# DeepGraphLearning/ULTRA

Measured on AMD Instinct MI355X. Metric: triples scored/sec (all-tail ranking) on FB15k237, higher is better.
Workload: dtype f32

## Files before the change

ultra_amd/build.py:

```python
import concurrent.futures as cf
import glob
import os
import subprocess
import sys

HERE = os.path.dirname(os.path.abspath(__file__))
CSRC = os.path.join(HERE, "csrc")
LIB_DIR = os.path.join(HERE, "lib")
OBJ_DIR = os.path.join(LIB_DIR, "obj")
LIB = os.path.join(LIB_DIR, "libultra_amd.so")
INCLUDE = os.path.join(os.path.dirname(HERE), "include")

HIPCC = os.environ.get("HIPCC", "/opt/rocm/bin/hipcc")
ARCH = "gfx950"
CFLAGS = ["--offload-arch=" + ARCH, "-O3", "-std=c++17", "-fPIC", "-ffp-contract=off",
          "-munsafe-fp-atomics", "-Wall", "-Wno-unused-function", "-I" + INCLUDE]


def _sources():
    return sorted(glob.glob(os.path.join(CSRC, "*.hip")) + glob.glob(os.path.join(CSRC, "*.cpp")))


def _headers_mtime():
    hs = glob.glob(os.path.join(CSRC, "*.hpp")) + glob.glob(os.path.join(INCLUDE, "*.h"))
    return max(os.path.getmtime(h) for h in hs)


def _compile(src, obj):
    cmd = [HIPCC] + CFLAGS + ["-c", src, "-o", obj]
    if src.endswith(".cpp"):
        cmd = [HIPCC] + CFLAGS + ["-x", "hip", "-c", src, "-o", obj]
    r = subprocess.run(cmd, capture_output=True, text=True)
    if r.returncode != 0:
        raise RuntimeError("hipcc failed for %s:\n%s\n%s" % (src, r.stdout, r.stderr))
    return r.stderr


def build(force=False, verbose=False):
    os.makedirs(OBJ_DIR, exist_ok=True)
    hm = _headers_mtime()
    jobs = []
    objs = []
    for src in _sources():
        obj = os.path.join(OBJ_DIR, os.path.basename(src) + ".o")
        objs.append(obj)
        stale = force or not os.path.exists(obj) or os.path.getmtime(obj) < max(os.path.getmtime(src), hm)
        if stale:
            jobs.append((src, obj))
    if jobs:
        with cf.ThreadPoolExecutor(max_workers=min(8, os.cpu_count() or 1)) as ex:
            futs = {ex.submit(_compile, s, o): s for s, o in jobs}
            for f in cf.as_completed(futs):
                warn = f.result()
                if verbose and warn.strip():
# ... 52 lines not shown
```

ultra_amd/csrc/plan.cpp:

```cpp
#include "plan.hpp"

#include <algorithm>
#include <cstdio>
#include <cstdlib>
#include <cstring>
#include <numeric>
#include <queue>

namespace ultra {

static thread_local std::string g_last_error;

void set_error(const std::string &msg) { g_last_error = msg; }

static int bits_for(int64_t n) {
    int b = 0;
    while ((int64_t(1) << b) < n) ++b;
    return b;
}

static void counting_pass(std::vector<int32_t> &order, const int32_t *key, int64_t nkey) {
    const int64_t n = (int64_t)order.size();
    std::vector<int64_t> start((size_t)nkey + 1, 0);
    for (int64_t i = 0; i < n; ++i) start[(size_t)key[order[i]] + 1]++;
// ... 102 lines not shown
            const int32_t t = p->type[(size_t)k], r = p->erow[(size_t)k];
            if (last_row[(size_t)t] != r) {
                last_row[(size_t)t] = r;
                ++runs;
            }
        }
        p->n_type_run = runs;
    }

    if (exact) {
        p->rec.resize((size_t)E * 2);
        for (int64_t k = 0; k < E; ++k) {
            p->rec[(size_t)2 * k] = p->col[(size_t)k];
            p->rec[(size_t)2 * k + 1] = p->type[(size_t)k];
        }
    }

    std::vector<Item> witems, gitems, chain;
    int32_t next_slot = 0;
    p->split_ptr.push_back(0);
    for (int64_t r = 0; r < num_out; ++r) {
        const int32_t b = p->row_ptr[(size_t)r], e = p->row_ptr[(size_t)r + 1];
        const int32_t deg = e - b;
        if (type_runs) {
            std::vector<Item> mine;
            int32_t pos = b;
            while (pos < e) {
                int32_t end = pos + 1;
                while (end < e && p->type[(size_t)end] == p->type[(size_t)pos]) ++end;
                const int32_t len_run = end - pos;
// ... 207 lines not shown
            sload[(size_t)stream] += p->items[(size_t)g].len + 1;
            scost[(size_t)stream] += p->items[(size_t)g].len + 1 + (walkers == 12 ? ROW_COST_12[(stream % ORDER_GROUPS) / 16] : 0.0);
        };
        {
        for (int64_t g = 0; g < nstream; ++g)
            if (weight[(size_t)g] > 0.0) sheap.push(Slot(1.0 / weight[(size_t)g], g));
        for (int64_t g = 0; g < n_item; ++g) {
            if (g < n_chain && !to_stream[(size_t)g]) continue;
            const Slot sl = sheap.top();
            sheap.pop();
            deal_into(sl.second, g);
            sheap.push(Slot((scost[(size_t)sl.second] + 1.0) / weight[(size_t)sl.second], sl.second));
        }
        }
        s->sdesc.assign((size_t)nstream * 2, 0);
        s->srec.reserve((size_t)(2 * (int64_t)steps) + 2 * ORDER_PAD);
        for (int64_t g = 0; g < nstream; ++g) {
            s->sdesc[(size_t)2 * g] = (int32_t)(s->srec.size() / 2);
            s->sdesc[(size_t)2 * g + 1] = (int32_t)sload[(size_t)g];
            s->max_stream_steps = std::max<int32_t>(s->max_stream_steps, (int32_t)sload[(size_t)g]);
            static const int row_order_env = std::getenv("ULTRA_STREAM_ROW_ORDER") ? std::atoi(std::getenv("ULTRA_STREAM_ROW_ORDER")) : -1;
            const int row_order = row_order_env >= 0 ? row_order_env : (walkers == 12 ? 2 : 0);
            std::sort(srows[(size_t)g].begin(), srows[(size_t)g].end(), [&](int32_t a, int32_t b) {
                const Item &ia = p->items[(size_t)a], &ib = p->items[(size_t)b];
                if (row_order == 1 && ia.len != ib.len) return ia.len > ib.len;
                if (row_order == 2 && ia.len != ib.len) return ia.len < ib.len;
                return ia.row < ib.row;
            });
            const int shift = (walkers == 12 && ULTRA_STREAM_PRESHIFT) ? 8 : 0;
            s->rec_shift = shift;
            for (int32_t it : srows[(size_t)g]) {
                const Item &row = p->items[(size_t)it];
                for (int32_t e = row.begin; e < row.begin + row.len; ++e) {
                    s->srec.push_back((int32_t)((uint32_t)p->col[(size_t)e] << shift));
                    s->srec.push_back((int32_t)((uint32_t)p->type[(size_t)e] << shift));
                }
                s->srec.push_back((int32_t)((uint32_t)row.row << shift));
                s->srec.push_back((int32_t)((uint32_t)p->num_rel << shift));
            }
        }
        s->srec_pad = 2 * ((int64_t)ORDER_PAD + (int64_t)s->max_stream_steps);
        s->srec.resize(s->srec.size() + (size_t)s->srec_pad, 0);
        s->prow_ptr.assign((size_t)nparts + 1, 0);
        for (int32_t q = 0; q < nparts; ++q) {
            std::vector<int32_t> mine;
            for (int32_t c : part_chain[(size_t)q]) mine.push_back(p->items[(size_t)c].row);
            for (int g = 0; g < ORDER_GROUPS; ++g)
                for (int32_t it : srows[(size_t)q * ORDER_GROUPS + g]) mine.push_back(p->items[(size_t)it].row);
            std::sort(mine.begin(), mine.end());
            s->prow.insert(s->prow.end(), mine.begin(), mine.end());
            while (s->prow.size() % 32) s->prow.push_back(-1);
            s->prow_ptr[(size_t)q + 1] = (int32_t)s->prow.size();
            s->max_rows = std::max<int32_t>(s->max_rows, (int32_t)mine.size());
            s->max_chain_rows = std::max<int32_t>(s->max_chain_rows, (int32_t)part_chain[(size_t)q].size());
        }
    }
// ... 62 lines not shown
        set_error("ultra_plan_get_info: NULL argument");
        return ULTRA_ERR_INVALID;
    }
    info->num_edge = p->num_edge;
    info->num_node = p->num_out;
    info->num_relation = p->num_rel;
    info->n_item = (int64_t)p->items.size();
    info->n_wave_item = p->n_w;
    info->n_group_item = p->n_g;
    info->n_unit = p->n_unit;
    info->n_split_row = (int64_t)p->split_row.size();
    info->n_partial_slot = p->n_slot;
    info->seg_len = p->seg_len;
    info->g_max = p->g_max;
    info->flags = p->flags;
    info->packed = p->packed_ok ? 1 : 0;
    info->on_device = p->on_device ? 1 : 0;
    info->has_transpose = (p->tplan && p->rplan) ? 1 : 0;
    info->n_type_run = p->n_type_run;
    info->dense_bytes = (int64_t)p->a_frag.size();
    info->n_chain_row = p->n_chain;
    info->dense_order_bytes = (int64_t)p->a_ex.size();
    return ULTRA_OK;
}

int32_t ultra_plan_export(const ultra_plan *p, int32_t which, void *dst, int64_t capacity, int64_t *count) {
    if (!p || !count) {
        set_error("ultra_plan_export: NULL argument");
        return ULTRA_ERR_INVALID;
    }
    const void *src = nullptr;
// ... 26 lines not shown
```

ultra_amd/csrc/plan.hpp:

```cpp
#pragma once

#include <cstdint>
#include <map>
#include <mutex>
#include <string>
#include <vector>

#include "../../include/ultra_rspmm.h"

namespace ultra {

struct Item {
    int32_t row, begin, len, slot;
};

struct Chunk {
    int32_t row, begin, count, flags;
};
enum { CHUNK_FIRST = 1, CHUNK_LAST = 2, CHUNK_LEN_SHIFT = 2 };
#ifndef ULTRA_ORDER_WAVES
#define ULTRA_ORDER_WAVES 16
#endif
constexpr int ORDER_WAVES = ULTRA_ORDER_WAVES;
constexpr int CHAIN_SLOTS = 4 * (ORDER_WAVES - 1);
constexpr int ORDER_GROUPS = 4 * ORDER_WAVES;
constexpr int CHUNK_PAD = 32;
#ifndef ULTRA_STREAM_PRESHIFT
#define ULTRA_STREAM_PRESHIFT 1
#endif
constexpr int ORDER_PAD = 128;

struct Schedule {
    int32_t nparts = 0;
    std::vector<int32_t> chunk_ptr, unit_ptr, units;
    std::vector<Chunk> chunks;
    std::vector<int32_t> srec, sdesc;
    std::vector<int32_t> prow, prow_ptr;
    int32_t *d_chunk_ptr = nullptr, *d_unit_ptr = nullptr, *d_units = nullptr, *d_srec = nullptr, *d_sdesc = nullptr;
    int32_t *d_prow = nullptr, *d_prow_ptr = nullptr;
    Chunk *d_chunks = nullptr;
    double max_cost = 0.0, mean_cost = 0.0;
    int32_t max_rows = 0;
    int32_t max_chain_rows = 0;
    int32_t max_stream_steps = 0;
    int32_t rec_shift = 0;
    int64_t srec_pad = 2 * ORDER_PAD;
};

struct WeightCopy {
    void *buf = nullptr;
    size_t bytes = 0;
    int64_t epoch = 0;
    const void *src = nullptr;
    int32_t dtype = -1;
    void *stream = nullptr;
    unsigned long long cap_id = 0;
};

struct DevicePlan {
    int32_t *row_ptr = nullptr, *col = nullptr, *type = nullptr, *perm = nullptr, *erow = nullptr;
    int32_t *rec = nullptr;
    uint32_t *packed = nullptr;
    Item *items = nullptr;
    int32_t *split_row = nullptr, *split_ptr = nullptr;
    uint8_t *a_frag = nullptr;
    uint8_t *a16 = nullptr;
    uint8_t *a_ex = nullptr;
    uint8_t *self_loop = nullptr;
    WeightCopy w_copy[2];
    void *partial = nullptr;
    size_t partial_bytes = 0;
    void *rb_rec_c = nullptr, *rb_seg_c = nullptr, *rb_multi_c = nullptr;
    void *rb_rec_t = nullptr, *rb_seg_t = nullptr, *rb_multi_t = nullptr;
    void *rb_work = nullptr;
    size_t rb_work_bytes = 0;
    int device = -1;
// ... 9 lines not shown
    int64_t num_edge = 0, num_out = 0, num_in = 0, num_rel = 0;
    int32_t seg_len = 256, g_max = 64, flags = 0;
    int32_t type_bits = 0;
    bool packed_ok = false;
    int32_t max_row_len = -1;
    bool rb_built = false;
    int64_t rb_n_seg_c = 0, rb_n_multi_c = 0, rb_n_part_c = 0, rb_n_seg_t = 0, rb_n_multi_t = 0, rb_n_part_t = 0;

    std::vector<int32_t> row_ptr, col, type, perm, erow;
    std::vector<uint32_t> packed;
    std::vector<ultra::Item> items;
    int64_t n_w = 0, n_g = 0, n_unit = 0;
    int64_t n_chain = 0;
    int32_t chain_min = 256;
    std::vector<int32_t> rec;
    std::map<int32_t, ultra::Schedule *> schedules;
    std::mutex sched_mu;
    std::vector<int32_t> split_row, split_ptr;
    int64_t n_slot = 0;
    int64_t n_type_run = 0;

    std::vector<uint8_t> a_frag;
    int32_t dense_rt = 0, dense_kg = 0, dense_tc = 0, dense_ntc = 0;
    bool dense_overflow = false;
    std::vector<uint8_t> a16;
    int32_t a16_chunks = 0;
    std::vector<uint8_t> a_ex;

    std::vector<uint8_t> self_loop;

// ... 20 lines not shown
```

ultra_amd/csrc/rspmm_api.hip:

```cpp
#include <hip/hip_runtime.h>

#include <cstdio>
#include <cstring>
#include <functional>
#include <string>
#include <vector>

#include "device_scope.hpp"
#include "layer0_kernels.hpp"
#include "rspmm_bwd_kernels.hpp"
#include "rspmm_kernels.hpp"
#include "rspmm_order_kernels.hpp"
#include "rspmm_rows_kernels.hpp"
#include "rows_bwd_kernels.hpp"

namespace ultra {

#define ULTRA_EXTERN_VARIANT(T_, VEC_, MODE_) \
    template <>                               \
    hipError_t launch_fwd_variant<T_, VEC_, MODE_>(int, int, const FwdParams &, int, int, size_t, hipStream_t);
ULTRA_EXTERN_VARIANT(float, 4, 0)
ULTRA_EXTERN_VARIANT(float, 1, 0)
ULTRA_EXTERN_VARIANT(float, 4, 1)
ULTRA_EXTERN_VARIANT(float, 4, 2)
// ... 114 lines not shown
    if (p->flags & ULTRA_PLAN_DENSE) {
        if ((rc = upload_array(&p->d.a_frag, p->a_frag))) return rc;
        if (!p->a16.empty() && (rc = upload_array(&p->d.a16, p->a16))) return rc;
        if (!p->a_ex.empty() && (rc = upload_array(&p->d.a_ex, p->a_ex))) return rc;
        p->d.device = dev;
        p->on_device = true;
        return ULTRA_OK;
    }
    if ((rc = upload_array(&p->d.row_ptr, p->row_ptr))) return rc;
    if ((rc = upload_array(&p->d.col, p->col))) return rc;
    if ((rc = upload_array(&p->d.type, p->type))) return rc;
    if (p->flags & ULTRA_PLAN_EXACT_ORDER) {
        int64_t longest = 0;
        for (size_t i = (size_t)p->n_chain; i < p->items.size(); ++i) longest = std::max<int64_t>(longest, p->items[i].len);
        const size_t pad = (size_t)ORDER_PAD + (size_t)std::min<int64_t>(longest, 1 << 20);
        std::vector<int32_t> perm_pad(p->perm), rec_pad(p->rec);
        perm_pad.resize(p->perm.size() + pad, 0);
        rec_pad.resize(p->rec.size() + 2 * pad, 0);
        if ((rc = upload_array(&p->d.perm, perm_pad))) return rc;
        if ((rc = upload_array(&p->d.rec, rec_pad))) return rc;
    } else if ((rc = upload_array(&p->d.perm, p->perm))) {
        return rc;
    }
    if ((rc = upload_array(&p->d.erow, p->erow))) return rc;
    if ((rc = upload_array(&p->d.packed, p->packed))) return rc;
    if ((rc = upload_array(&p->d.items, p->items))) return rc;
    if ((rc = upload_array(&p->d.split_row, p->split_row))) return rc;
    if ((rc = upload_array(&p->d.split_ptr, p->split_ptr))) return rc;
    if (!p->self_loop.empty() && (rc = upload_array(&p->d.self_loop, p->self_loop))) return rc;
    p->d.device = dev;
    p->on_device = true;
    return ULTRA_OK;
}

static void free_schedules(ultra_plan *p) {
    std::lock_guard<std::mutex> lock(p->sched_mu);
    for (auto &kv : p->schedules) {
        Schedule *s = kv.second;
        if (s->d_chunk_ptr) (void)hipFree(s->d_chunk_ptr);
        if (s->d_unit_ptr) (void)hipFree(s->d_unit_ptr);
        if (s->d_units) (void)hipFree(s->d_units);
        if (s->d_chunks) (void)hipFree(s->d_chunks);
        if (s->d_srec) (void)hipFree(s->d_srec);
        if (s->d_sdesc) (void)hipFree(s->d_sdesc);
        if (s->d_prow) (void)hipFree(s->d_prow);
        if (s->d_prow_ptr) (void)hipFree(s->d_prow_ptr);
        delete s;
// ... 22 lines not shown
    *out = s;
    return ULTRA_OK;
}

static void free_device(ultra_plan *p) {
    free_schedules(p);
    if (!p->on_device) return;
    (void)hipFree(p->d.row_ptr);
    (void)hipFree(p->d.col);
    (void)hipFree(p->d.type);
    (void)hipFree(p->d.perm);
    (void)hipFree(p->d.erow);
    (void)hipFree(p->d.packed);
    (void)hipFree(p->d.items);
    if (p->d.rec) (void)hipFree(p->d.rec);
    (void)hipFree(p->d.split_row);
    (void)hipFree(p->d.split_ptr);
    if (p->d.a_frag) (void)hipFree(p->d.a_frag);
    if (p->d.a16) (void)hipFree(p->d.a16);
    if (p->d.a_ex) (void)hipFree(p->d.a_ex);
    if (p->d.self_loop) (void)hipFree(p->d.self_loop);
    for (WeightCopy &c : p->d.w_copy)
        if (c.buf) (void)hipFree(c.buf);
    if (p->d.partial) (void)hipFree(p->d.partial);
    for (void *q : {p->d.rb_rec_c, p->d.rb_seg_c, p->d.rb_multi_c, p->d.rb_rec_t, p->d.rb_seg_t, p->d.rb_multi_t, p->d.rb_work})
        if (q) (void)hipFree(q);
    p->rb_built = false;
    p->d = DevicePlan();
    p->on_device = false;
}
// ... 153 lines not shown
    op->upd.mode = 1;
    *lds = std::max(*lds, (size_t)UPDATE_LDS_FLOATS * sizeof(float));
    Schedule *sched12 = nullptr;
    const bool pitch_ok = !ULTRA_STREAM_PRESHIFT || op->x_row_bytes == 256u;
    const bool walk_heavy = (double)(p->num_edge + p->num_out) >= 10.0 * (double)p->num_out;
    const bool want3 = update_form() == 3 || (update_form() == 0 && walk_heavy);
    if (want3 && pitch_ok && ORDER_WAVES == 16 && upd->out_stride_row * (int64_t)sizeof(float) == (int64_t)op->x_row_bytes) {
        if ((rc = get_schedule(p, op->nparts, &sched12, ORDER_WALKERS))) return rc;
        const size_t overlay = std::max(ring_bytes, (size_t)UPD2_OVERLAY_BYTES);
        const size_t need = rel_bytes + overlay + UPD2_CTL_BYTES;
        if (need <= di.lds_optin && sched12->max_chain_rows <= UPD2_MAX_CHAIN_ROWS) {
            op->upd.mode = 3;
            op->max_stream_steps = sched12->max_stream_steps;
            op->upd.ctl_off = (uint32_t)(rel_bytes + overlay);
            op->srec = sched12->d_srec;
            op->sdesc = reinterpret_cast<const int2 *>(sched12->d_sdesc);
            op->chunk_ptr = sched12->d_chunk_ptr;
            op->chunks = reinterpret_cast<const int4 *>(sched12->d_chunks);
            *lds = need;
        }
    }
    if (update_form() == 2) {
        set_error("ultra_rspmm_forward_update: update form 2 (rows by reference) was removed in ABI 6; ask for 0 (the library's "
                  "choice), 1 (tail) or 3 (beside the walk, rows through LDS)");
        return ULTRA_ERR_UNSUPPORTED;
    }
    if (update_form() >= 2 && op->upd.mode != update_form()) {
        set_error("ultra_rspmm_forward_update: the update beside the walk does not fit this call (LDS / rows per workgroup)");
        return ULTRA_ERR_UNSUPPORTED;
    }
// ... 40 lines not shown
                         const ultra_mat *out, hipStream_t stream, const FwdCall &call, const FwdParams &fp, const DevInfo &di,
                         size_t ring_bytes, bool point_fill) {
    const size_t esz = dtype == ULTRA_F32 ? 4 : 8;
    const int64_t row_len = out->row_len;
    const int64_t *bnd_rows = call.bnd_rows;
    int rc;
    const size_t rel_bytes = (mul != BIN_RHS) ? (size_t)(p->num_rel + 1) * 64 * esz : 0;
    const bool rel_lds = g_tuning.rel_lds != 0 && rel_bytes > 0 && rel_bytes + ring_bytes <= di.lds_optin;
    const int grid = launch_grid(di);
    OrderParams op;
    std::memset(&op, 0, sizeof(op));
    op.smod = std::min<int32_t>(fp.n_span, grid);
    op.nparts = grid / op.smod;
    Schedule *sched = nullptr;
    if ((rc = get_schedule(p, op.nparts, &sched))) return rc;
    op.rec = p->d.rec;
    op.perm = p->d.perm;
    op.w = w;
    op.items = reinterpret_cast<const int4 *>(p->d.items);
    op.unit_ptr = sched->d_unit_ptr;
    op.units = sched->d_units;
    op.chunk_ptr = sched->d_chunk_ptr;
    op.chunks = reinterpret_cast<const int4 *>(sched->d_chunks);
    op.n_chain = (int32_t)p->n_chain;
    op.n_item = (int32_t)p->items.size();
    op.rel = fp.rel, op.x = fp.x, op.bnd = fp.bnd;
    op.bnd_rows = fp.bnd_rows;
    op.bnd_fill_on = point_fill ? 1 : 0;
    op.bnd_fill = 0.f;
    op.out = fp.out;
    op.out_stride_outer = fp.out_stride_outer, op.out_stride_row = fp.out_stride_row;
    op.n_outer = fp.n_outer, op.row_len = fp.row_len, op.spans_per_outer = fp.spans_per_outer, op.n_span = fp.n_span;
    op.num_rel = fp.num_rel;
    op.has_bnd = fp.has_bnd;
    op.has_chain = p->n_chain > 0 ? 1 : 0;
    op.keep_mode = fp.keep_mode;
    op.w_stride_outer = (w && call.w_samples) ? (int32_t)call.w_stride_outer : 0;
    op.x_row_bytes = fp.x_row_bytes, op.rel_row_bytes = fp.rel_row_bytes;
    op.trace = g_order_trace;
    op.err = device_error_word();
    op.srec = sched->d_srec;
    op.sdesc = reinterpret_cast<const int2 *>(sched->d_sdesc);
    op.use_streams = (unit_walk() == 0 && dtype == ULTRA_F32 && rel_lds && !w && (mul == BIN_MUL || mul == BIN_ADD) &&
                      row_len % 64 == 0 && (!bnd || bnd_rows) && out->stride_row == x->stride_row &&
                      p->num_out <= p->num_in && (uint64_t)p->num_out * (uint64_t)out->stride_row * esz < (1ull << 32))
                         ? 1
                         : 0;
    size_t lds = (rel_lds ? rel_bytes : 0) + ring_bytes;
    if (call.upd && (rc = choose_update_form(p, call.upd, sched, di, rel_bytes, ring_bytes, &op, &lds))) return rc;
    if (call.ev_before) HIP_TRY(hipEventRecord(call.ev_before, stream));
#define ULTRA_ORDER_LAUNCH(T_)                                                                          \
    (rel_lds ? (w ? launch_order_variant<T_, true, true>(sum, mul, op, grid, lds, stream)                \
                  : launch_order_variant<T_, true, false>(sum, mul, op, grid, lds, stream))              \
             : (w ? launch_order_variant<T_, false, true>(sum, mul, op, grid, lds, stream)               \
                  : launch_order_variant<T_, false, false>(sum, mul, op, grid, lds, stream)))
    const hipError_t e = dtype == ULTRA_F32 ? ULTRA_ORDER_LAUNCH(float) : ULTRA_ORDER_LAUNCH(double);
#undef ULTRA_ORDER_LAUNCH
    if (e != hipSuccess) return hip_fail(e, "rspmm_order_kernel launch");
    if (call.ev_after) HIP_TRY(hipEventRecord(call.ev_after, stream));
    return ULTRA_OK;
}

static int forward_walk(ultra_plan *p, int sum, int mul, int dtype, const void *w, const ultra_mat *bnd, const ultra_mat *out,
                        hipStream_t stream, const FwdCall &call, FwdParams &fp, const DevInfo &di, int VEC, bool rot_far) {
// ... 1034 lines not shown

int32_t ultra_plan_schedule_export(ultra_plan *plan, int32_t nparts, int32_t which, int32_t *dst, int64_t capacity, int64_t *count) {
    const int32_t walkers = (nparts & ULTRA_SCHEDULE_12_WALKERS) ? 12 : 16;
    nparts &= ~ULTRA_SCHEDULE_12_WALKERS;
    if (!plan || !count || nparts <= 0) return invalid("ultra_plan_schedule_export: bad argument");
    if (!(plan->flags & ULTRA_PLAN_EXACT_ORDER)) return invalid("schedules belong to ULTRA_PLAN_EXACT_ORDER plans");
    Schedule *s = build_schedule(plan, nparts, walkers);
    const int32_t *src = nullptr;
    int64_t n = 0;
    switch (which) {
        case 0: src = s->chunk_ptr.data(), n = (int64_t)s->chunk_ptr.size(); break;
        case 1: src = s->unit_ptr.data(), n = (int64_t)s->unit_ptr.size(); break;
        case 2: src = s->units.data(), n = (int64_t)s->units.size(); break;
        case 3: src = reinterpret_cast<const int32_t *>(s->chunks.data()), n = (int64_t)s->chunk_ptr.back() * 4; break;
        case 4: src = s->sdesc.data(), n = (int64_t)s->sdesc.size(); break;
        case 5: src = s->srec.data(), n = (int64_t)s->srec.size() - s->srec_pad; break;
        case 6: src = s->prow.data(), n = (int64_t)s->prow.size(); break;
        case 7: src = s->prow_ptr.data(), n = (int64_t)s->prow_ptr.size(); break;
        default: delete s; return invalid("ultra_plan_schedule_export: unknown array id");
    }
    *count = n;
    int rc = ULTRA_OK;
    if (dst) {
        if (capacity < n) rc = invalid("ultra_plan_schedule_export: destination too small");
        else if (n) std::memcpy(dst, src, (size_t)n * sizeof(int32_t));
        if (rc == ULTRA_OK && which == 5 && s->rec_shift)
            for (int64_t i = 0; i < n; ++i) dst[i] = (int32_t)((uint32_t)dst[i] >> s->rec_shift);
    }
    delete s;
    return rc;
}

int32_t ultra_device_error(void) { return take_device_error(); }

int32_t ultra_set_tuning(const ultra_tuning *t) {
    if (!t) {
        g_tuning = ultra_tuning{0, 0, -1, -1, 0, {0, 0, 0}};
        return ULTRA_OK;
    }
// ... 57 lines not shown
```

ultra_amd/csrc/rspmm_order_kernels.hpp:

```cpp
#pragma once

#include "rspmm_kernels.hpp"
#ifdef ULTRA_ORDER_ASM_HEADER
#include ULTRA_ORDER_ASM_HEADER
#else
#include "rspmm_order_asm.hpp"
#endif
#include "update_tile.hpp"

static_assert(ULTRA_STREAM_PRESHIFT_GEN == ULTRA_STREAM_PRESHIFT,
              "the generated walk and plan.cpp must agree on the record format of the twelve-walker schedules (plan.hpp)");

#pragma clang fp contract(off)

namespace ultra {

constexpr int ORDER_THREADS = 64 * ORDER_WAVES;
constexpr uint32_t SPIN_CAP = 1u << 20;
enum { ORDER_SPIN_LOOK = 1,
       ORDER_SPIN_MEET = 2,
       ORDER_SPIN_CHAIN_WALKER = 3,
       ORDER_SPIN_CHAIN_UPDATER = 4,
       ORDER_SPIN_PARK = 5 };
constexpr int ORDER_UPDATERS = 4, ORDER_WALKERS = ORDER_THREADS / 64 - ORDER_UPDATERS;
#ifndef ULTRA_CHAIN_PRIO
#define ULTRA_CHAIN_PRIO 1
#endif
static_assert(CHAIN_SLOTS == 4 * (ORDER_THREADS / 64 - 1), "one ring slot per producer group");

struct OrderParams {
    const int32_t *rec;
    const int32_t *perm;
    const void *w;
    const int4 *items;
    const int32_t *unit_ptr, *units, *chunk_ptr;
    const int4 *chunks;
    const int32_t *srec;
    const int2 *sdesc;
    int32_t use_streams;
    int32_t n_chain, n_item;
    MatArg rel, x, bnd;
    const long long *bnd_rows;
    int32_t bnd_fill_on;
    float bnd_fill;
    void *out;
    long long out_stride_outer, out_stride_row;
    int32_t n_outer, row_len, spans_per_outer, n_span;
    int32_t num_rel, has_bnd, has_chain;
    int32_t keep_mode;
    int32_t smod, nparts;
    uint32_t x_row_bytes, rel_row_bytes;
    long long *trace;
    uint32_t *err;
// ... 253 lines not shown
#else
#define ULTRA_ORDER_VGPR_CAP
#endif
#ifndef ULTRA_UPD_SIMDS
#define ULTRA_UPD_SIMDS 4
#endif
__device__ __forceinline__ int order_role(const int pw) {
#if ULTRA_UPD_SIMDS == 2 && ULTRA_ORDER_WAVES == 16
    return pw < 10 ? pw : (pw == 12 ? 10 : pw == 13 ? 11 : pw == 10 ? 12 : pw == 11 ? 13 : pw);
#elif ULTRA_UPD_SIMDS == 1 && ULTRA_ORDER_WAVES == 16
    return (pw & 3) == 3 ? 12 + (pw >> 2) : 3 * (pw >> 2) + (pw & 3);
#else
    return pw;
#endif
}
template <typename T, int SUM, int MUL, bool REL_LDS, bool WEIGHTED, bool STREAMS, int UPDATE = 0>
__global__ void __launch_bounds__(ORDER_THREADS) ULTRA_ORDER_VGPR_CAP rspmm_order_kernel(const OrderParams p) {
    static_assert(!STREAMS || OrderAsm<T, MUL, REL_LDS, WEIGHTED>::value, "group streams exist for the assembly configurations only");
    static_assert(!UPDATE || (STREAMS && sizeof(T) == 4), "the layer update follows the fp32 stream walk");
    static_assert(UPDATE != 3 || ORDER_UPDATERS == 4, "form 3 splits the 64 output features over four update waves");
    constexpr int SPAN = 64;
    using P = Pack<T, 4>;
    using V = typename VecOf<T, 4>::type;
    extern __shared__ __attribute__((aligned(16))) unsigned char smem[];
    T *lds_rel = reinterpret_cast<T *>(smem);
    T *ring = lds_rel + ((REL_LDS && MUL != BIN_RHS) ? (size_t)(p.num_rel + 1) * SPAN : 0);

    const int tid = threadIdx.x;
    const int lane = tid & 63;
    const int wave = order_role(rfl(tid >> 6));
    constexpr int nwave = ORDER_THREADS / 64;
    const int part = blockIdx.x / p.smod;
// ... 162 lines not shown
#endif
#if ULTRA_CHAIN_PRIO
                __builtin_amdgcn_s_setprio(0);
#endif
            } else {
                const int slot = (wave - 1) * 4 + grp;
                const auto chunk_begin = [&](const int ci) {
                    return load_uniform(reinterpret_cast<const int32_t *>(p.chunks + min(ci, c1 - 1)) + 1);
                };
#if ULTRA_DBG_CHAIN == 2
                if constexpr (true) {
                    for (int k = c0; k < c1; ++k) __syncthreads();
                } else
#endif
                if constexpr (STREAMS && ULTRA_ASM_PRODUCE) {
                    order_produce_asm<MUL>(c1 - c0, p.chunks + c0, (uint32_t)slot * 8u, lane_bytes, lds_addr(lds_rel_lane),
                                           lds_addr(ring) + (uint32_t)((wave - 1) * 64 + lane) * 16u, xbase,
                                           reinterpret_cast<const char *>(p.rec), p.x_row_bytes);
                } else {
                    const int2 *recs = reinterpret_cast<const int2 *>(p.rec) + slot;
                    const int32_t *perm = p.perm + slot;
                    struct Rec {
                        int c, t;
                        T w;
                    };
                    const auto load_rec = [&](const int b) {
                        const int2 ct = recs[b];
                        Rec r;
                        r.c = ct.x, r.t = ct.y, r.w = T(1);
                        if (WEIGHTED) r.w = wt[perm[b]];
                        return r;
                    };
                    const auto gather = [&](const Rec &r) {
// ... 81 lines not shown
                if (p.has_bnd) {
                    const P b = *reinterpret_cast<const P *>(reinterpret_cast<const T *>(p.bnd.ptr) + outer * p.bnd.stride_outer + d0);
#pragma unroll
                    for (int e = 0; e < 4; ++e) bv[e] = b.v[e];
                    bndoff = (uint32_t)bnd_row * p.x_row_bytes + lane_bytes;
                }
                const float bz = (SUM != 0 && p.bnd_fill_on) ? p.bnd_fill : (SUM == 1 ? __builtin_inff() : -__builtin_inff());
                constexpr int POST = UPDATE == 3 ? 2 : 0;
#if ULTRA_STREAM_DIET
                const int l8_arg = len - (l16 & 7);
                const uint32_t rmk = (uint32_t)p.num_rel << ((POST != 0 && ULTRA_STREAM_PRESHIFT_GEN) ? 8 : 0);
#else
                const int l8_arg = l16 & 7;
                const uint32_t rmk = 0;
#endif
                if (ns > 0)
                    order_stream_asm<SUM, MUL, POST>(len, (uint32_t)(sd.x + (l16 & 7)) * 8u, l8_arg, lane_bytes, lds_addr(lds_rel_lane),
                                                     lds_addr(lds_rel_lane) + (uint32_t)p.num_rel * 256u, bndoff, bv, bz, ns, nf, xbase,
                                                     reinterpret_cast<const char *>(p.srec),
                                                     reinterpret_cast<const char *>(reinterpret_cast<const T *>(p.out) + outer * p.out_stride_outer),
                                                     p.x_row_bytes, lds_addr(const_cast<uint32_t *>(ctl)), lds_addr(ring), rmk);
                if constexpr (UPDATE == 3) {
                    asm volatile("" ::: "memory");
                    if (lane == 0 && ctl[UPD2_CTL_ERR] != 0) report_spin(ORDER_SPIN_PARK);
                    if (lane == 0) __hip_atomic_fetch_add(const_cast<uint32_t *>(ctl) + 1, 1u, __ATOMIC_RELAXED, __HIP_MEMORY_SCOPE_WORKGROUP);
                }
            }
            if constexpr (UPDATE == 3) {
                if (wave >= ORDER_WALKERS) {
                    using f32x4m = float __attribute__((ext_vector_type(4)));
                    int lane_u = lane;
                    asm volatile("" : "+v"(lane_u));
                    const int u = wave - ORDER_WALKERS;
                    const int i16 = lane_u & 15, kk = lane_u >> 4;
                    using lds_f = __attribute__((address_space(3))) float;
                    using lds_f4 = __attribute__((address_space(3))) f32x4m;
// ... 325 lines not shown
                *reinterpret_cast<P *>(dst) = acc;
            }
        }
        }
    }
    if (p.trace) {
        __syncthreads();
        if (tid == 0) p.trace[3 * blockIdx.x + 2] = clock64();
        if constexpr (UPDATE == 3) {
            if (tid == 0) p.trace[24 * gridDim.x + blockIdx.x] = ctl[UPD2_CTL_RETRIES];
        }
    }
}

template <typename T, int SUM, int MUL, bool REL_LDS, bool WEIGHTED, bool STREAMS, int UPDATE = 0>
inline hipError_t launch_order_inst(const OrderParams &p, int grid, size_t lds, hipStream_t s) {
    auto kern = rspmm_order_kernel<T, SUM, MUL, REL_LDS, WEIGHTED, STREAMS, UPDATE>;
    static size_t lds_opted_in = 0;
    if (lds > 48 * 1024 && lds > lds_opted_in) {
        hipError_t e = hipFuncSetAttribute(reinterpret_cast<const void *>(kern), hipFuncAttributeMaxDynamicSharedMemorySize, (int)lds);
        if (e != hipSuccess) return e;
        lds_opted_in = lds;
    }
    hipLaunchKernelGGL(kern, dim3(grid), dim3(ORDER_THREADS), lds, s, p);
    return hipGetLastError();
}
template <typename T, int SUM, int MUL, bool REL_LDS, bool WEIGHTED>
inline hipError_t launch_order_one(const OrderParams &p, int grid, size_t lds, hipStream_t s) {
    if constexpr (OrderAsm<T, MUL, REL_LDS, WEIGHTED>::value) {
        if constexpr (sizeof(T) == 4) {
            if (p.use_streams && p.upd.weight)
                return p.upd.mode == 3 ? launch_order_inst<T, SUM, MUL, REL_LDS, WEIGHTED, true, 3>(p, grid, lds, s)
                                       : launch_order_inst<T, SUM, MUL, REL_LDS, WEIGHTED, true, 1>(p, grid, lds, s);
// ... 30 lines not shown
```

ultra_amd/rspmm.py:

```python
import copy
import ctypes
import sys
from collections import OrderedDict, namedtuple

import torch
from torch import autograd

from . import _lib, tasks
from .data import Data
from ._lib import UltraMat, check, lib, ptr, stream_of

module = sys.modules[__name__]

_DTYPES = {torch.float32: _lib.F32, torch.float64: _lib.F64}


_WEIGHT_EPOCH = [0]
DENSE_RELATION_GRAD = True


def tag_edge_weight(edge_weight):
    _WEIGHT_EPOCH[0] += 1
    edge_weight._ultra_epoch = (_WEIGHT_EPOCH[0], edge_weight._version)
    return edge_weight
# ... 150 lines not shown
                if torch.cuda.is_available():
                    torch.cuda.synchronize()
                lib.ultra_plan_destroy(h)
            except Exception:
                pass
            self._h = None

    def pin(self, delta=1):
        for p in (self, self.typed, self.dense, self._dense_t):
            if p is not None and getattr(p, "_h", None):
                check(lib.ultra_plan_pin(p._h, int(delta)))

    def info(self):
        info = _lib.PlanInfo()
        check(lib.ultra_plan_get_info(self._h, ctypes.byref(info)))
        return {name: getattr(info, name) for name, _ in _lib.PlanInfo._fields_}

    def schedule_info(self, nparts):
        info = _lib.ScheduleInfo()
        check(lib.ultra_plan_schedule_info(self._h, int(nparts), ctypes.byref(info)))
        return {name: getattr(info, name) for name, _ in _lib.ScheduleInfo._fields_ if name != "reserved"}

    def _export(self, fn, *key):
        n = ctypes.c_int64()
        check(fn(self._h, *key, None, 0, ctypes.byref(n)))
        out = torch.empty(n.value, dtype=torch.int32)
        check(fn(self._h, *key, out.data_ptr(), n.value, ctypes.byref(n)))
        return out

    def schedule(self, nparts):
        out = [self._export(lib.ultra_plan_schedule_export, int(nparts), which) for which in range(4)]
# ... 1054 lines not shown
```

Before: 213.5 million.

## Pack edge records into 4-byte words for the stream and producer walks

Edge records (column id and relation type) are now packed into one 32-bit word, with the type in the low bits, whenever the bit widths fit. The packing applies to both the per-plan record array and the twelve-walker stream schedules. New generated assembly loops unpack these words, and a separate kernel instantiation is selected when packing is on. The goal is to halve the record bandwidth and footprint in the gather walk, at the cost of extra shift and mask instructions, a second kernel variant, and a build-time code generator dependency.

```diff
diff --git a/ultra_amd/build.py b/ultra_amd/build.py
--- a/ultra_amd/build.py
+++ b/ultra_amd/build.py
@@ -13,16 +13,25 @@
 
 HIPCC = os.environ.get("HIPCC", "/opt/rocm/bin/hipcc")
 ARCH = "gfx950"
+GEN_DIR = os.path.join(LIB_DIR, "gen")
 CFLAGS = ["--offload-arch=" + ARCH, "-O3", "-std=c++17", "-fPIC", "-ffp-contract=off",
-          "-munsafe-fp-atomics", "-Wall", "-Wno-unused-function", "-I" + INCLUDE]
+          "-munsafe-fp-atomics", "-Wall", "-Wno-unused-function", "-I" + INCLUDE, "-I" + GEN_DIR]
 
 
 def _sources():
     return sorted(glob.glob(os.path.join(CSRC, "*.hip")) + glob.glob(os.path.join(CSRC, "*.cpp")))
 
 
+def _generate():
+    import importlib.util
+    spec = importlib.util.spec_from_file_location("ultra_gen_order_asm", os.path.join(os.path.dirname(HERE), "tools", "gen_order_asm.py"))
+    gen = importlib.util.module_from_spec(spec)
+    spec.loader.exec_module(gen)
+    gen.main_packed(os.path.join(GEN_DIR, "rspmm_order_asm_packed.hpp"), quiet=True)
+
+
 def _headers_mtime():
-    hs = glob.glob(os.path.join(CSRC, "*.hpp")) + glob.glob(os.path.join(INCLUDE, "*.h"))
+    hs = glob.glob(os.path.join(CSRC, "*.hpp")) + glob.glob(os.path.join(INCLUDE, "*.h")) + glob.glob(os.path.join(GEN_DIR, "*.hpp"))
     return max(os.path.getmtime(h) for h in hs)
 
 
@@ -38,6 +47,7 @@
 
 def build(force=False, verbose=False):
     os.makedirs(OBJ_DIR, exist_ok=True)
+    _generate()
     hm = _headers_mtime()
     jobs = []
     objs = []
diff --git a/ultra_amd/csrc/plan.cpp b/ultra_amd/csrc/plan.cpp
--- a/ultra_amd/csrc/plan.cpp
+++ b/ultra_amd/csrc/plan.cpp
@@ -140,6 +140,10 @@
             p->rec[(size_t)2 * k] = p->col[(size_t)k];
             p->rec[(size_t)2 * k + 1] = p->type[(size_t)k];
         }
+        const char *env = std::getenv("ULTRA_RECORD_BYTES");
+        const bool want = env ? std::atoi(env) == 4 : ULTRA_RECORDS_PACKED_DEFAULT != 0;
+        const int tb = bits_for(num_rel + 1), id_bits = bits_for(std::max<int64_t>(std::max(num_in, num_out), 1));
+        p->rec_tb = (want && ULTRA_STREAM_PRESHIFT && tb + id_bits <= 32) ? tb : 0;
     }
 
     std::vector<Item> witems, gitems, chain;
@@ -377,9 +381,12 @@
         }
         }
         s->sdesc.assign((size_t)nstream * 2, 0);
-        s->srec.reserve((size_t)(2 * (int64_t)steps) + 2 * ORDER_PAD);
+        const int tb = (walkers == 12 && ULTRA_STREAM_PRESHIFT) ? p->rec_tb : 0;
+        const int rec_words = tb ? 1 : 2;
+        s->rec_tb = tb;
+        s->srec.reserve((size_t)(rec_words * ((int64_t)steps + ORDER_PAD)));
         for (int64_t g = 0; g < nstream; ++g) {
-            s->sdesc[(size_t)2 * g] = (int32_t)(s->srec.size() / 2);
+            s->sdesc[(size_t)2 * g] = (int32_t)(s->srec.size() / rec_words);
             s->sdesc[(size_t)2 * g + 1] = (int32_t)sload[(size_t)g];
             s->max_stream_steps = std::max<int32_t>(s->max_stream_steps, (int32_t)sload[(size_t)g]);
             static const int row_order_env = std::getenv("ULTRA_STREAM_ROW_ORDER") ? std::atoi(std::getenv("ULTRA_STREAM_ROW_ORDER")) : -1;
@@ -391,9 +398,15 @@
                 return ia.row < ib.row;
             });
             const int shift = (walkers == 12 && ULTRA_STREAM_PRESHIFT) ? 8 : 0;
-            s->rec_shift = shift;
+            s->rec_shift = tb ? 0 : shift;
             for (int32_t it : srows[(size_t)g]) {
                 const Item &row = p->items[(size_t)it];
+                if (tb) {
+                    for (int32_t e = row.begin; e < row.begin + row.len; ++e)
+                        s->srec.push_back((int32_t)(((uint32_t)p->col[(size_t)e] << tb) | (uint32_t)p->type[(size_t)e]));
+                    s->srec.push_back((int32_t)(((uint32_t)row.row << tb) | (uint32_t)p->num_rel));
+                    continue;
+                }
                 for (int32_t e = row.begin; e < row.begin + row.len; ++e) {
                     s->srec.push_back((int32_t)((uint32_t)p->col[(size_t)e] << shift));
                     s->srec.push_back((int32_t)((uint32_t)p->type[(size_t)e] << shift));
@@ -402,7 +415,7 @@
                 s->srec.push_back((int32_t)((uint32_t)p->num_rel << shift));
             }
         }
-        s->srec_pad = 2 * ((int64_t)ORDER_PAD + (int64_t)s->max_stream_steps);
+        s->srec_pad = rec_words * ((int64_t)ORDER_PAD + (int64_t)s->max_stream_steps);
         s->srec.resize(s->srec.size() + (size_t)s->srec_pad, 0);
         s->prow_ptr.assign((size_t)nparts + 1, 0);
         for (int32_t q = 0; q < nparts; ++q) {
@@ -495,7 +508,7 @@
     info->seg_len = p->seg_len;
     info->g_max = p->g_max;
     info->flags = p->flags;
-    info->packed = p->packed_ok ? 1 : 0;
+    info->packed = (p->packed_ok ? 1 : 0) | (p->rec_tb << 8);
     info->on_device = p->on_device ? 1 : 0;
     info->has_transpose = (p->tplan && p->rplan) ? 1 : 0;
     info->n_type_run = p->n_type_run;
diff --git a/ultra_amd/csrc/plan.hpp b/ultra_amd/csrc/plan.hpp
--- a/ultra_amd/csrc/plan.hpp
+++ b/ultra_amd/csrc/plan.hpp
@@ -28,6 +28,9 @@
 #ifndef ULTRA_STREAM_PRESHIFT
 #define ULTRA_STREAM_PRESHIFT 1
 #endif
+#ifndef ULTRA_RECORDS_PACKED_DEFAULT
+#define ULTRA_RECORDS_PACKED_DEFAULT 1
+#endif
 constexpr int ORDER_PAD = 128;
 
 struct Schedule {
@@ -44,6 +47,7 @@
     int32_t max_chain_rows = 0;
     int32_t max_stream_steps = 0;
     int32_t rec_shift = 0;
+    int32_t rec_tb = 0;
     int64_t srec_pad = 2 * ORDER_PAD;
 };
 
@@ -60,6 +64,7 @@
 struct DevicePlan {
     int32_t *row_ptr = nullptr, *col = nullptr, *type = nullptr, *perm = nullptr, *erow = nullptr;
     int32_t *rec = nullptr;
+    uint32_t *rec4 = nullptr;
     uint32_t *packed = nullptr;
     Item *items = nullptr;
     int32_t *split_row = nullptr, *split_ptr = nullptr;
@@ -99,6 +104,8 @@
     int64_t n_chain = 0;
     int32_t chain_min = 256;
     std::vector<int32_t> rec;
+    int32_t rec_tb = 0;
+    size_t rec_pad = 0;
     std::map<int32_t, ultra::Schedule *> schedules;
     std::mutex sched_mu;
     std::vector<int32_t> split_row, split_ptr;
diff --git a/ultra_amd/csrc/rspmm_api.hip b/ultra_amd/csrc/rspmm_api.hip
--- a/ultra_amd/csrc/rspmm_api.hip
+++ b/ultra_amd/csrc/rspmm_api.hip
@@ -152,11 +152,15 @@
         int64_t longest = 0;
         for (size_t i = (size_t)p->n_chain; i < p->items.size(); ++i) longest = std::max<int64_t>(longest, p->items[i].len);
         const size_t pad = (size_t)ORDER_PAD + (size_t)std::min<int64_t>(longest, 1 << 20);
-        std::vector<int32_t> perm_pad(p->perm), rec_pad(p->rec);
+        std::vector<int32_t> perm_pad(p->perm);
         perm_pad.resize(p->perm.size() + pad, 0);
-        rec_pad.resize(p->rec.size() + 2 * pad, 0);
         if ((rc = upload_array(&p->d.perm, perm_pad))) return rc;
-        if ((rc = upload_array(&p->d.rec, rec_pad))) return rc;
+        p->rec_pad = pad;
+        if (p->rec_tb == 0) {
+            std::vector<int32_t> rec8(p->rec);
+            rec8.resize(p->rec.size() + 2 * pad, 0);
+            if ((rc = upload_array(&p->d.rec, rec8))) return rc;
+        }
     } else if ((rc = upload_array(&p->d.perm, p->perm))) {
         return rc;
     }
@@ -169,6 +173,19 @@
     p->d.device = dev;
     p->on_device = true;
     return ULTRA_OK;
+}
+
+static int upload_records(ultra_plan *p, bool packed) {
+    std::lock_guard<std::mutex> lock(p->sched_mu);
+    if (packed ? p->d.rec4 != nullptr : p->d.rec != nullptr) return ULTRA_OK;
+    if (packed) {
+        std::vector<uint32_t> rec4(p->col.size() + p->rec_pad, 0u);
+        for (size_t k = 0; k < p->col.size(); ++k) rec4[k] = ((uint32_t)p->col[k] << p->rec_tb) | (uint32_t)p->type[k];
+        return upload_array(&p->d.rec4, rec4);
+    }
+    std::vector<int32_t> rec8(p->rec);
+    rec8.resize(p->rec.size() + 2 * p->rec_pad, 0);
+    return upload_array(&p->d.rec, rec8);
 }
 
 static void free_schedules(ultra_plan *p) {
@@ -221,6 +238,7 @@
     (void)hipFree(p->d.packed);
     (void)hipFree(p->d.items);
     if (p->d.rec) (void)hipFree(p->d.rec);
+    if (p->d.rec4) (void)hipFree(p->d.rec4);
     (void)hipFree(p->d.split_row);
     (void)hipFree(p->d.split_ptr);
     if (p->d.a_frag) (void)hipFree(p->d.a_frag);
@@ -404,6 +422,7 @@
             op->max_stream_steps = sched12->max_stream_steps;
             op->upd.ctl_off = (uint32_t)(rel_bytes + overlay);
             op->srec = sched12->d_srec;
+            op->srec_tb = sched12->rec_tb;
             op->sdesc = reinterpret_cast<const int2 *>(sched12->d_sdesc);
             op->chunk_ptr = sched12->d_chunk_ptr;
             op->chunks = reinterpret_cast<const int4 *>(sched12->d_chunks);
@@ -474,7 +493,6 @@
     op.nparts = grid / op.smod;
     Schedule *sched = nullptr;
     if ((rc = get_schedule(p, op.nparts, &sched))) return rc;
-    op.rec = p->d.rec;
     op.perm = p->d.perm;
     op.w = w;
     op.items = reinterpret_cast<const int4 *>(p->d.items);
@@ -500,6 +518,7 @@
     op.trace = g_order_trace;
     op.err = device_error_word();
     op.srec = sched->d_srec;
+    op.srec_tb = sched->rec_tb;
     op.sdesc = reinterpret_cast<const int2 *>(sched->d_sdesc);
     op.use_streams = (unit_walk() == 0 && dtype == ULTRA_F32 && rel_lds && !w && (mul == BIN_MUL || mul == BIN_ADD) &&
                       row_len % 64 == 0 && (!bnd || bnd_rows) && out->stride_row == x->stride_row &&
@@ -508,6 +527,13 @@
                          : 0;
     size_t lds = (rel_lds ? rel_bytes : 0) + ring_bytes;
     if (call.upd && (rc = choose_update_form(p, call.upd, sched, di, rel_bytes, ring_bytes, &op, &lds))) return rc;
+    const bool producers_packed = op.use_streams && p->rec_tb > 0 && ULTRA_ASM_PRODUCE;
+    if ((rc = upload_records(p, producers_packed))) return rc;
+    op.rec = p->d.rec;
+    op.rec4 = p->d.rec4;
+    op.rec_tb = producers_packed ? p->rec_tb : 0;
+    if ((op.srec_tb > 0) != (op.rec_tb > 0 && call.upd && op.upd.mode == 3))
+        return invalid("rspmm_order_kernel: the schedule's record format does not match the plan's");
     if (call.ev_before) HIP_TRY(hipEventRecord(call.ev_before, stream));
 #define ULTRA_ORDER_LAUNCH(T_)                                                                          \
     (rel_lds ? (w ? launch_order_variant<T_, true, true>(sum, mul, op, grid, lds, stream)                \
@@ -1572,7 +1598,7 @@
         case 2: src = s->units.data(), n = (int64_t)s->units.size(); break;
         case 3: src = reinterpret_cast<const int32_t *>(s->chunks.data()), n = (int64_t)s->chunk_ptr.back() * 4; break;
         case 4: src = s->sdesc.data(), n = (int64_t)s->sdesc.size(); break;
-        case 5: src = s->srec.data(), n = (int64_t)s->srec.size() - s->srec_pad; break;
+        case 5: src = s->srec.data(), n = ((int64_t)s->srec.size() - s->srec_pad) * (s->rec_tb ? 2 : 1); break;
         case 6: src = s->prow.data(), n = (int64_t)s->prow.size(); break;
         case 7: src = s->prow_ptr.data(), n = (int64_t)s->prow_ptr.size(); break;
         default: delete s; return invalid("ultra_plan_schedule_export: unknown array id");
@@ -1581,6 +1607,11 @@
     int rc = ULTRA_OK;
     if (dst) {
         if (capacity < n) rc = invalid("ultra_plan_schedule_export: destination too small");
+        else if (which == 5 && s->rec_tb)
+            for (int64_t i = 0; i < n / 2; ++i) {
+                const uint32_t r = (uint32_t)src[i];
+                dst[2 * i] = (int32_t)(r >> s->rec_tb), dst[2 * i + 1] = (int32_t)(r & ((1u << s->rec_tb) - 1u));
+            }
         else if (n) std::memcpy(dst, src, (size_t)n * sizeof(int32_t));
         if (rc == ULTRA_OK && which == 5 && s->rec_shift)
             for (int64_t i = 0; i < n; ++i) dst[i] = (int32_t)((uint32_t)dst[i] >> s->rec_shift);
diff --git a/ultra_amd/csrc/rspmm_order_kernels.hpp b/ultra_amd/csrc/rspmm_order_kernels.hpp
--- a/ultra_amd/csrc/rspmm_order_kernels.hpp
+++ b/ultra_amd/csrc/rspmm_order_kernels.hpp
@@ -6,10 +6,14 @@
 #else
 #include "rspmm_order_asm.hpp"
 #endif
+#include "rspmm_order_asm_packed.hpp"
 #include "update_tile.hpp"
 
 static_assert(ULTRA_STREAM_PRESHIFT_GEN == ULTRA_STREAM_PRESHIFT,
               "the generated walk and plan.cpp must agree on the record format of the twelve-walker schedules (plan.hpp)");
+
+static_assert(ULTRA_STREAM_PACKED_GEN || !ULTRA_STREAM_PRESHIFT,
+              "plan.cpp packs the records of the pre-shifted schedules: the generated walk must have the loops that unpack them");
 
 #pragma clang fp contract(off)
 
@@ -37,6 +41,8 @@
     const int4 *chunks;
     const int32_t *srec;
     const int2 *sdesc;
+    const uint32_t *rec4;
+    int32_t rec_tb, srec_tb;
     int32_t use_streams;
     int32_t n_chain, n_item;
     MatArg rel, x, bnd;
@@ -320,8 +326,9 @@
     return pw;
 #endif
 }
-template <typename T, int SUM, int MUL, bool REL_LDS, bool WEIGHTED, bool STREAMS, int UPDATE = 0>
-__global__ void __launch_bounds__(ORDER_THREADS) ULTRA_ORDER_VGPR_CAP rspmm_order_kernel(const OrderParams p) {
+template <typename T, int SUM, int MUL, bool REL_LDS, bool WEIGHTED, bool STREAMS, int UPDATE, bool REC4>
+__device__ __forceinline__ void order_kernel_body(const OrderParams &p) {
+    static_assert(!REC4 || STREAMS, "packed records are read by the generated loops of the stream kernels");
     static_assert(!STREAMS || OrderAsm<T, MUL, REL_LDS, WEIGHTED>::value, "group streams exist for the assembly configurations only");
     static_assert(!UPDATE || (STREAMS && sizeof(T) == 4), "the layer update follows the fp32 stream walk");
     static_assert(UPDATE != 3 || ORDER_UPDATERS == 4, "form 3 splits the 64 output features over four update waves");
@@ -514,9 +521,14 @@
                 } else
 #endif
                 if constexpr (STREAMS && ULTRA_ASM_PRODUCE) {
-                    order_produce_asm<MUL>(c1 - c0, p.chunks + c0, (uint32_t)slot * 8u, lane_bytes, lds_addr(lds_rel_lane),
-                                           lds_addr(ring) + (uint32_t)((wave - 1) * 64 + lane) * 16u, xbase,
-                                           reinterpret_cast<const char *>(p.rec), p.x_row_bytes);
+                    const uint32_t ring_lane_addr = lds_addr(ring) + (uint32_t)((wave - 1) * 64 + lane) * 16u;
+                    if constexpr (REC4)
+                        order_produce_asm_packed<MUL>(c1 - c0, p.chunks + c0, (uint32_t)slot * 4u, lane_bytes, lds_addr(lds_rel_lane),
+                                                      ring_lane_addr, xbase, reinterpret_cast<const char *>(p.rec4), p.x_row_bytes,
+                                                      (uint32_t)p.rec_tb, (1u << p.rec_tb) - 1u);
+                    else
+                        order_produce_asm<MUL>(c1 - c0, p.chunks + c0, (uint32_t)slot * 8u, lane_bytes, lds_addr(lds_rel_lane),
+                                               ring_lane_addr, xbase, reinterpret_cast<const char *>(p.rec), p.x_row_bytes);
                 } else {
                     const int2 *recs = reinterpret_cast<const int2 *>(p.rec) + slot;
                     const int32_t *perm = p.perm + slot;
@@ -628,12 +640,22 @@
                 const int l8_arg = l16 & 7;
                 const uint32_t rmk = 0;
 #endif
-                if (ns > 0)
-                    order_stream_asm<SUM, MUL, POST>(len, (uint32_t)(sd.x + (l16 & 7)) * 8u, l8_arg, lane_bytes, lds_addr(lds_rel_lane),
-                                                     lds_addr(lds_rel_lane) + (uint32_t)p.num_rel * 256u, bndoff, bv, bz, ns, nf, xbase,
-                                                     reinterpret_cast<const char *>(p.srec),
-                                                     reinterpret_cast<const char *>(reinterpret_cast<const T *>(p.out) + outer * p.out_stride_outer),
-                                                     p.x_row_bytes, lds_addr(const_cast<uint32_t *>(ctl)), lds_addr(ring), rmk);
+                const uint32_t mark = lds_addr(lds_rel_lane) + (uint32_t)p.num_rel * 256u;
+                const char *const srec = reinterpret_cast<const char *>(p.srec);
+                const char *const obase = reinterpret_cast<const char *>(reinterpret_cast<const T *>(p.out) + outer * p.out_stride_outer);
+                const uint32_t rec_index = (uint32_t)(sd.x + (l16 & 7));
+                if (ns > 0) {
+#if ULTRA_STREAM_PACKED_GEN
+                    if constexpr (REC4 && POST == 2)
+                        order_stream_asm_packed<SUM, MUL>(len, rec_index * 4u, l8_arg, lane_bytes, lds_addr(lds_rel_lane), mark, bndoff, bv,
+                                                          bz, ns, nf, xbase, srec, obase, p.x_row_bytes, lds_addr(const_cast<uint32_t *>(ctl)),
+                                                          lds_addr(ring), rmk, (uint32_t)p.srec_tb, (1u << p.srec_tb) - 1u);
+                    else
+#endif
+                        order_stream_asm<SUM, MUL, POST>(len, rec_index * 8u, l8_arg, lane_bytes, lds_addr(lds_rel_lane), mark, bndoff, bv, bz,
+                                                         ns, nf, xbase, srec, obase, p.x_row_bytes, lds_addr(const_cast<uint32_t *>(ctl)),
+                                                         lds_addr(ring), rmk);
+                }
                 if constexpr (UPDATE == 3) {
                     asm volatile("" ::: "memory");
                     if (lane == 0 && ctl[UPD2_CTL_ERR] != 0) report_spin(ORDER_SPIN_PARK);
@@ -989,9 +1011,24 @@
 }
 
 template <typename T, int SUM, int MUL, bool REL_LDS, bool WEIGHTED, bool STREAMS, int UPDATE = 0>
+__global__ void __launch_bounds__(ORDER_THREADS) ULTRA_ORDER_VGPR_CAP rspmm_order_kernel(const OrderParams p) {
+    order_kernel_body<T, SUM, MUL, REL_LDS, WEIGHTED, STREAMS, UPDATE, false>(p);
+}
+namespace packed_records {
+template <typename T, int SUM, int MUL, bool REL_LDS, bool WEIGHTED, bool STREAMS, int UPDATE = 0>
+__global__ void __launch_bounds__(ORDER_THREADS) ULTRA_ORDER_VGPR_CAP rspmm_order_kernel(const OrderParams p) {
+    order_kernel_body<T, SUM, MUL, REL_LDS, WEIGHTED, STREAMS, UPDATE, true>(p);
+}
+}
+
+template <typename T, int SUM, int MUL, bool REL_LDS, bool WEIGHTED, bool STREAMS, int UPDATE = 0>
 inline hipError_t launch_order_inst(const OrderParams &p, int grid, size_t lds, hipStream_t s) {
     auto kern = rspmm_order_kernel<T, SUM, MUL, REL_LDS, WEIGHTED, STREAMS, UPDATE>;
-    static size_t lds_opted_in = 0;
+    if constexpr (STREAMS) {
+        if (p.rec_tb) kern = packed_records::rspmm_order_kernel<T, SUM, MUL, REL_LDS, WEIGHTED, STREAMS, UPDATE>;
+    }
+    static size_t lds_opted_in_of[2] = {0, 0};
+    size_t &lds_opted_in = lds_opted_in_of[(STREAMS && p.rec_tb) ? 1 : 0];
     if (lds > 48 * 1024 && lds > lds_opted_in) {
         hipError_t e = hipFuncSetAttribute(reinterpret_cast<const void *>(kern), hipFuncAttributeMaxDynamicSharedMemorySize, (int)lds);
         if (e != hipSuccess) return e;
diff --git a/ultra_amd/rspmm.py b/ultra_amd/rspmm.py
--- a/ultra_amd/rspmm.py
+++ b/ultra_amd/rspmm.py
@@ -188,7 +188,11 @@
     def info(self):
         info = _lib.PlanInfo()
         check(lib.ultra_plan_get_info(self._h, ctypes.byref(info)))
-        return {name: getattr(info, name) for name, _ in _lib.PlanInfo._fields_}
+        out = {name: getattr(info, name) for name, _ in _lib.PlanInfo._fields_}
+        out["record_type_bits"] = out["packed"] >> 8
+        out["record_bytes"] = 4 if out["record_type_bits"] else 8
+        out["packed"] &= 1
+        return out
 
     def schedule_info(self, nparts):
         info = _lib.ScheduleInfo()
```

Result: no change. 218.3 million (median of 6 runs) (+2.2%).
